# hpsim/OGL

Hardware: AMD Instinct MI355X
Metric: cg_iters_per_sec (higher is better)
Workload: dtype f64

## Files before the change

ogl_amd/csrc/kernels.hpp:

```cpp
#pragma once
#include <hip/hip_runtime.h>

#include "common.hpp"

namespace ogl {

struct DevCriterion {
    double tolerance, rel_tol;
    int32_t min_iter, max_iter, frequency, export_res;
};

struct DevScalars {
    double rho, prev_rho, beta;
    double alpha, omega, gamma;
    double norm_factor;
    double init_res, res;
    double xbar;
    double sums[4];
    int32_t iter;
    int32_t stop;
    int32_t n_evals;
    int32_t stop_phase;
    int32_t stop_turn;
    int32_t comm_error;
// ... 63 lines not shown
    const int32_t *chunk_bptr = nullptr;
    const int32_t *boundary_rows = nullptr;
    const int32_t *entry_ptrs = nullptr;
    const int32_t *cols = nullptr;
    const double *vals = nullptr;
    const double *recv = nullptr;
    const unsigned long long *local_flag = nullptr;
    int32_t n_neigh = 0;
    uint32_t seq = 0;
    long long timeout_ticks = 0;
    DevScalars *s = nullptr;
};
void launch_spmv(hipStream_t st, const DevCsr &A, int mode, const double *x, const double *b,
                 double *y, const SpmvDots &dots, const DevScalars *gate, const HaloFused &hf = HaloFused{});

struct DevEll {
    int32_t n_rows = 0;
    int32_t width = 0;
    int64_t stride = 0;
    const int32_t *cols = nullptr;
    const double *vals = nullptr;
    bool stream = false;
};
void launch_spmv_ell(hipStream_t st, const DevEll &A, int mode, const double *x, const double *b,
                     double *y, const SpmvDots &dots, const DevScalars *gate, const HaloFused &hf = HaloFused{});
struct DevSell {
    int32_t n_rows = 0;
    const SellChunk *chunks = nullptr;
    const int32_t *dict = nullptr;
    const uint8_t *codes = nullptr;
    const double *vals = nullptr;
    const int32_t *spill_chunk_ptr = nullptr, *spill_rows = nullptr, *spill_ptrs = nullptr, *spill_cols = nullptr;
    const double *spill_vals = nullptr;
    bool stream = false;
    int32_t xcd_group = 0;
    const uint16_t *rmap = nullptr;
    const int32_t *block_order = nullptr;
    int32_t n_blocks = 0;
};
void launch_spmv_sell(hipStream_t st, const DevSell &A, int mode, const double *x, const double *b,
                      double *y, const SpmvDots &dots, const DevScalars *gate, const HaloFused &hf = HaloFused{});
struct DevSym {
    int32_t n_rows = 0;
    int32_t nd = 0;
    int32_t d[4] = {0, 0, 0, 0};
    const uint8_t *mask = nullptr;
    const double *planes = nullptr;
    bool stream = false;
    const int32_t *block_order = nullptr;
    int32_t n_blocks = 0;
};
void launch_spmv_sym(hipStream_t st, const DevSym &A, int mode, const double *x, const double *b, double *y,
                     const SpmvDots &dots, const DevScalars *gate, const HaloFused &hf = HaloFused{});
struct DevSymx {
    int32_t n_rows = 0;
    const SymxChunk *chunks = nullptr, *chunks_general = nullptr;
    int32_t n_blocks_general = 0;
    const uint8_t *mask = nullptr;
    const double *planes = nullptr;
    const int32_t *ex_rowptr = nullptr, *ex_cols = nullptr;
    const int32_t *ex_lrow = nullptr;
    const double *ex_vals = nullptr;
    bool stream = false;
    bool fast = false;
    int32_t xcd_group = 0;
    int32_t n_blocks = 0;
};
void launch_spmv_symx(hipStream_t st, const DevSymx &A, int mode, const double *x, const double *b, double *y,
                      const SpmvDots &dots, const DevScalars *gate, const HaloFused &hf = HaloFused{});
void launch_gather_coeffs_masked(hipStream_t st, int64_t n, const int32_t *map, const double *source,
                                 double *out);
void launch_gather_sell(hipStream_t st, int32_t n_chunks, const SellChunk *chunks, const int32_t *map,
                        const double *source, double *out);

void launch_spmv_non_local(hipStream_t st, const DevHalo &H, int mode, const double *recv,
                           double *y, const DevScalars *gate);
void launch_pack(hipStream_t st, const DevHalo &H, const double *x, double *send,
                 const DevScalars *gate);

void launch_gather_coeffs(hipStream_t st, int32_t nnz, const int32_t *ldu_mapping,
                          const double *source, double *coeffs);
void launch_jacobi_generate(hipStream_t st, const DevCsr &A, double *inv_diag);
void launch_jacobi_generate_pos(hipStream_t st, const DevCsr &A, const int32_t *diag_pos, double *inv_diag);
void launch_jacobi_generate_diag(hipStream_t st, int32_t n_rows, const double *diag, double *inv_diag);

struct DevBlockJacobi {
    int32_t n_rows = 0;
    int32_t n_blocks = 0;
    int32_t stride = 0;
    const int32_t *block_ptrs = nullptr;
    const int32_t *row_block = nullptr;
    double *blocks = nullptr;
    int32_t uniform = 0;
    const int32_t *rows = nullptr, *pos = nullptr;
    int32_t by_device_row = 0;
    int32_t perm_xcd_group = 0;
};
constexpr int MAX_JACOBI_BLOCK = 32;
void launch_bj_generate(hipStream_t st, const DevCsr &A, const DevBlockJacobi &J,
                        bool group_lanes = true);
void launch_bj_apply(hipStream_t st, const DevBlockJacobi &J, const double *in, double *out,
                     double *dot_part, const DevScalars *gate);
void launch_bj_apply_staged(hipStream_t st, const DevBlockJacobi &J, const double *in, double *out, double *dot_part,
                            const DevScalars *gate, double *tmp_in, double *tmp_out);

constexpr int ISAI_THREAD_ROW = 32;
// ... 334 lines not shown
```

ogl_amd/csrc/kernels_spmv_sym.hip:

```cpp
#include <algorithm>

#include "device_common.hpp"
#include "resident_cg_turn.hpp"

namespace ogl {

namespace {

struct SymOffsets {
    int d[SYM_MAX_OFFSETS];
};
SymOffsets sym_offsets(const DevSym &A, bool *fast)
{
    SymOffsets off;
    for (int j = 0; j < SYM_MAX_OFFSETS; ++j) off.d[j] = A.d[j];
    *fast = A.nd >= 2 && A.d[1] == 1;
    for (int j = 2; j < A.nd; ++j) *fast = *fast && (A.d[j] % 2 == 0);
    return off;
}
template <int MODE, int ND, bool FAST, bool STREAM>
__device__ __forceinline__ double2 sym_rows(int chunk, const RowPair &rp, int n_rows, const SymOffsets &off,
                                            const uint8_t *__restrict__ mask, const double *__restrict__ planes,
                                            const double *__restrict__ x, const double *__restrict__ b,
                                            double2 &xd_out)
{
    const int t = threadIdx.x;
    const int row = rp.row;
    const unsigned mm = *reinterpret_cast<const unsigned short *>(mask + row);
    const unsigned m0 = mm & 0xffu, m1 = mm >> 8;
    double2 acc;
    acc.x = acc.y = 0.0;
    if (MODE == SPMV_RESIDUAL) acc = ld2(b, rp);
    double2 up[ND];
    const double *own = planes + (long)chunk * (ND * CHUNK_ROWS) + t * ROWS_PER_THREAD;
#pragma unroll
    for (int j = 0; j < ND; ++j)
        up[j] = (STREAM && (j == 0 || (FAST && j == 1))) ? ld_pair_stream(own + (long)j * CHUNK_ROWS)
                                                         : *reinterpret_cast<const double2 *>(own + (long)j * CHUNK_ROWS);
    const double2 xd = xd_out = ld2(x, rp);
    const int last = n_rows - 1, last_pair = last & ~1;
    double2 lo[ND];
#pragma unroll
    for (int j = 1; j < ND; ++j) {
        const int r0 = max(row - off.d[j], 0), r1 = max(row + 1 - off.d[j], 0);
        const long a0 = (long)(r0 >> 9) * (ND * CHUNK_ROWS) + (long)j * CHUNK_ROWS + (r0 & (CHUNK_ROWS - 1));
        const long a1 = (long)(r1 >> 9) * (ND * CHUNK_ROWS) + (long)j * CHUNK_ROWS + (r1 & (CHUNK_ROWS - 1));
        if (FAST && j >= 2) {
            lo[j] = *reinterpret_cast<const double2 *>(planes + a0);
        } else if (FAST) {
            if (STREAM) {
                lo[j].x = __shfl_up(up[1].y, 1, WAVE);
                if ((t & (WAVE - 1)) == 0) lo[j].x = planes[a0];
            } else {
                lo[j].x = planes[a0];
            }
            lo[j].y = up[1].x;
        } else {
            lo[j].x = planes[a0];
            lo[j].y = planes[a1];
        }
    }
    static_assert(CHUNK_ROWS == 512, "row >> 9 above");
    double2 xl[ND], xu[ND];
#pragma unroll
    for (int j = 1; j < ND; ++j) {
        if (FAST && j >= 2) {
            xl[j] = *reinterpret_cast<const double2 *>(x + min(max(row - off.d[j], 0), last_pair));
            xu[j] = *reinterpret_cast<const double2 *>(x + min(row + off.d[j], last_pair));
        } else if (FAST) {
            xl[j].x = x[min(max(row - 1, 0), last)];
            xl[j].y = xd.x;
            xu[j].x = xd.y;
            xu[j].y = x[min(row + 2, last)];
        } else {
            xl[j].x = x[min(max(row - off.d[j], 0), last)];
            xl[j].y = x[min(max(row + 1 - off.d[j], 0), last)];
            xu[j].x = x[min(row + off.d[j], last)];
            xu[j].y = x[min(row + 1 + off.d[j], last)];
        }
    }
#pragma unroll
    for (int j = ND - 1; j >= 1; --j) {
        if ((m0 >> (ND - 1 - j)) & 1u) {
            const double p = lo[j].x * xl[j].x;
            acc.x = (MODE == SPMV_RESIDUAL) ? acc.x - p : acc.x + p;
        }
        if ((m1 >> (ND - 1 - j)) & 1u) {
            const double p = lo[j].y * xl[j].y;
            acc.y = (MODE == SPMV_RESIDUAL) ? acc.y - p : acc.y + p;
        }
    }
    if ((m0 >> (ND - 1)) & 1u) {
        const double p = up[0].x * xd.x;
        acc.x = (MODE == SPMV_RESIDUAL) ? acc.x - p : acc.x + p;
    }
    if ((m1 >> (ND - 1)) & 1u) {
        const double p = up[0].y * xd.y;
        acc.y = (MODE == SPMV_RESIDUAL) ? acc.y - p : acc.y + p;
    }
#pragma unroll
    for (int j = 1; j < ND; ++j) {
        if ((m0 >> (ND - 1 + j)) & 1u) {
            const double p = up[j].x * xu[j].x;
            acc.x = (MODE == SPMV_RESIDUAL) ? acc.x - p : acc.x + p;
        }
        if ((m1 >> (ND - 1 + j)) & 1u) {
            const double p = up[j].y * xu[j].y;
            acc.y = (MODE == SPMV_RESIDUAL) ? acc.y - p : acc.y + p;
        }
    }
    return acc;
}

template <int MODE, int NDOT, int ND, bool FAST, bool STREAM>
__global__ __launch_bounds__(BLOCK) void k_spmv_sym(int n_rows, int n_chunks, SymOffsets off,
                                                    const uint8_t *__restrict__ mask,
                                                    const double *__restrict__ planes,
                                                    const double *__restrict__ x, const double *__restrict__ b,
                                                    double *__restrict__ y, const double *__restrict__ w,
                                                    double *__restrict__ dot_partials,
                                                    double *__restrict__ dot2_partials, const DevScalars *gate,
                                                    const int *__restrict__ block_order, HaloFused hf)
{
    __shared__ double slot[N_WAVES];
    __shared__ double ys[CHUNK_ROWS];
    if (gate && gate->stop) return;
    const int chunk = block_order ? block_order[blockIdx.x] : xcd_chunk(blockIdx.x);
    if (chunk < 0 || chunk >= n_chunks) return;
    const RowPair rp = my_rows(chunk, n_rows);
    double2 xd;
    double2 acc = sym_rows<MODE, ND, FAST, STREAM>(chunk, rp, n_rows, off, mask, planes, x, b, xd);
    if (hf.chunk_bptr) halo_fused_add<MODE>(hf, chunk, acc.x, acc.y, ys);
    st2(y, rp, acc);
    if (NDOT >= 1) {
        const double2 vw = ld2(w, rp);
        double d = 0.0, d2 = 0.0;
        if (rp.n > 0) {
            d += vw.x * acc.x;
            d2 += acc.x * acc.x;
        }
        if (rp.n > 1) {
            d += vw.y * acc.y;
            d2 += acc.y * acc.y;
        }
        const double s = block_sum(d, slot);
        if (threadIdx.x == 0) dot_partials[chunk] = s;
        if (NDOT >= 2) {
            const double s2 = block_sum(d2, slot);
            if (threadIdx.x == 0) dot2_partials[chunk] = s2;
        }
    }
}

template <int ND>
struct TurnSymRegs {
    double2 vd[2], vl[2][ND], vu[2][ND], up[ND], lo[ND];
};
template <int ND, bool FAST, bool STREAM>
__device__ __forceinline__ void turn_sym_load(TurnSymRegs<ND> &R, int chunk, const RowPair &rp, int n_rows,
                                              const SymOffsets &off, const double *__restrict__ planes,
                                              const double *__restrict__ p_in, const double *__restrict__ z)
{
    const int row = rp.row;
    const double *src[2] = {p_in, z};
    const int last = n_rows - 1, last_pair = last & ~1;
#pragma unroll
    for (int a = 0; a < 2; ++a) {
        const double *__restrict__ v = src[a];
        R.vd[a] = ld2(v, rp);
#pragma unroll
        for (int j = 1; j < ND; ++j) {
            if (FAST && j >= 2) {
                R.vl[a][j] = *reinterpret_cast<const double2 *>(v + min(max(row - off.d[j], 0), last_pair));
                R.vu[a][j] = *reinterpret_cast<const double2 *>(v + min(row + off.d[j], last_pair));
            } else if (FAST) {
                R.vl[a][j].x = v[min(max(row - 1, 0), last)];
                R.vl[a][j].y = R.vd[a].x;
                R.vu[a][j].x = R.vd[a].y;
                R.vu[a][j].y = v[min(row + 2, last)];
            } else {
                R.vl[a][j].x = v[min(max(row - off.d[j], 0), last)];
                R.vl[a][j].y = v[min(max(row + 1 - off.d[j], 0), last)];
                R.vu[a][j].x = v[min(row + off.d[j], last)];
                R.vu[a][j].y = v[min(row + 1 + off.d[j], last)];
            }
        }
    }
    const double *own = planes + (long)chunk * (ND * CHUNK_ROWS) + threadIdx.x * ROWS_PER_THREAD;
#pragma unroll
    for (int j = 0; j < ND; ++j)
        R.up[j] = (STREAM && (j == 0 || (FAST && j == 1))) ? ld_pair_stream(own + (long)j * CHUNK_ROWS)
                                                           : *reinterpret_cast<const double2 *>(own + (long)j * CHUNK_ROWS);
#pragma unroll
    for (int j = 1; j < ND; ++j) {
        const int r0 = max(row - off.d[j], 0), r1 = max(row + 1 - off.d[j], 0);
        const long a0 = (long)(r0 >> 9) * (ND * CHUNK_ROWS) + (long)j * CHUNK_ROWS + (r0 & (CHUNK_ROWS - 1));
        const long a1 = (long)(r1 >> 9) * (ND * CHUNK_ROWS) + (long)j * CHUNK_ROWS + (r1 & (CHUNK_ROWS - 1));
        if (FAST && j >= 2) {
            R.lo[j] = *reinterpret_cast<const double2 *>(planes + a0);
        } else if (FAST) {
            if (STREAM) {
                const double prev = __shfl_up(R.up[1].y, 1, WAVE);
// ... 292 lines not shown
    double beta;
    if (!turn_await_beta(a, ts, lds, beta)) return;
    resident_cg_turn<R, L, K>(src, a, ts, lds, z, f, beta);
}

}

void launch_spmv_sym(hipStream_t st, const DevSym &A, int mode, const double *x, const double *b, double *y,
                     const SpmvDots &dots, const DevScalars *gate, const HaloFused &hf)
{
    if (A.n_rows == 0) return;
    const int nc = (int)n_chunks(A.n_rows);
    const dim3 grid(A.block_order ? A.n_blocks : xcd_grid(nc)), block(BLOCK);
    bool fast;
    const SymOffsets off = sym_offsets(A, &fast);
#define OGL_SYM_K(MODE, NDOT, ND, FAST, STREAM)                                                                          \
    hipLaunchKernelGGL((k_spmv_sym<MODE, NDOT, ND, FAST, STREAM>), grid, block, 0, st, A.n_rows, nc, off, A.mask, A.planes, \
                       x, b, y, dots.with, dots.part, dots.part_yy, gate, A.block_order, hf)
#define OGL_SYM_ND(MODE, NDOT, ND)                   \
    do {                                             \
        if (fast && A.stream)                        \
            OGL_SYM_K(MODE, NDOT, ND, true, true);   \
        else if (fast)                               \
            OGL_SYM_K(MODE, NDOT, ND, true, false);  \
        else if (A.stream)                           \
            OGL_SYM_K(MODE, NDOT, ND, false, true);  \
        else                                         \
            OGL_SYM_K(MODE, NDOT, ND, false, false); \
    } while (0)
#define OGL_SYM(MODE, NDOT)                    \
    do {                                       \
        if (A.nd == 2)                         \
            OGL_SYM_ND(MODE, NDOT, 2);         \
        else if (A.nd == 3)                    \
            OGL_SYM_ND(MODE, NDOT, 3);         \
        else                                   \
            OGL_SYM_ND(MODE, NDOT, 4);         \
    } while (0)
    static_assert(SYM_MAX_OFFSETS == 4, "instantiations above");
    if (mode == SPMV_RESIDUAL) {
        OGL_SYM(SPMV_RESIDUAL, 0);
    } else if (dots.part && dots.part_yy) {
        OGL_SYM(SPMV_PLAIN, 2);
    } else if (dots.part) {
        OGL_SYM(SPMV_PLAIN, 1);
    } else {
        OGL_SYM(SPMV_PLAIN, 0);
    }
#undef OGL_SYM
#undef OGL_SYM_ND
#undef OGL_SYM_K
}

void launch_cg_turn_sym(hipStream_t st, const DevSym &A, const double *p_in, double *p_out, double *x, const double *z,
                        double *q, double *part_beta, const DevScalars *sin, DevScalars *sout,
                        const double *part_rho, const double *part_norm, double *history, int first, const LeadBox &lead)
{
    if (A.n_rows == 0) return;
    const int nc = (int)n_chunks(A.n_rows);
    const dim3 grid(A.block_order ? A.n_blocks : xcd_grid(nc)), block(BLOCK);
    const bool led = lead.box && nc >= 3 * FIN_WAVES;
    bool fast;
    const SymOffsets off = sym_offsets(A, &fast);
#define OGL_TURN_K(ND, FAST)                                                                                                  \
    do {                                                                                                                      \
        if (led)                                                                                                              \
            hipLaunchKernelGGL((k_cg_turn_sym<ND, FAST, true>), grid, block, 0, st, A.n_rows, nc, off, A.mask, A.planes, p_in, \
                               p_out, x, z, q, part_beta, sin, sout, part_rho, part_norm, nc, history, first, A.block_order,  \
                               lead);                                                                                         \
        else                                                                                                                  \
            hipLaunchKernelGGL((k_cg_turn_sym<ND, FAST, false>), grid, block, 0, st, A.n_rows, nc, off, A.mask, A.planes,     \
                               p_in, p_out, x, z, q, part_beta, sin, sout, part_rho, part_norm, nc, history, first,           \
                               A.block_order, LeadBox{});                                                                     \
    } while (0)
#define OGL_TURN_ND(ND)              \
    do {                             \
        if (fast)                    \
            OGL_TURN_K(ND, true);    \
        else                         \
            OGL_TURN_K(ND, false);   \
    } while (0)
    if (A.nd == 2)
        OGL_TURN_ND(2);
    else if (A.nd == 3)
        OGL_TURN_ND(3);
    else
        OGL_TURN_ND(4);
#undef OGL_TURN_ND
#undef OGL_TURN_K
}

void launch_cg_turn_sym_big(hipStream_t st, const DevSym &A, const double *p_in, double *p_out, double *x,
                            const double *z, double *q, double *part_beta, const DevScalars *s,
                            const HaloFused &hf, const double *p_halo_in, double *p_halo_out)
{
    if (A.n_rows == 0) return;
    const int nc = (int)n_chunks(A.n_rows);
    const dim3 grid(A.block_order ? A.n_blocks : xcd_grid(nc)), block(BLOCK);
    bool fast;
    const SymOffsets off = sym_offsets(A, &fast);
#define OGL_TURN_K(ND, FAST, STREAM)                                                                                \
    do {                                                                                                            \
        if (hf.chunk_bptr)                                                                                          \
            hipLaunchKernelGGL((k_cg_turn_sym_big<ND, FAST, STREAM, true>), grid, block, 0, st, A.n_rows, nc, off,  \
                               A.mask, A.planes, p_in, p_out, x, z, q, part_beta, s, A.block_order, hf, p_halo_in,  \
                               p_halo_out);                                                                         \
// ... 108 lines not shown
```

ogl_amd/csrc/solver.hpp:

```cpp
#pragma once
#include <hip/hip_runtime.h>

#include <algorithm>
#include <map>
#include <memory>
#include <string>
#include <vector>

#include "comm.hpp"
#include "common.hpp"
#include "host_matrix.hpp"
#include "kernels.hpp"
#include "setup_kernels.hpp"
#include "spmv_layouts.hpp"

namespace ogl {

struct MgLevel {
    int32_t n = 0, nnz = 0, n_coarse = 0;
    int passes = 0;
    bool own = true;
    DevBuf<int32_t> row_ptrs, cols;
    DevBuf<double> vals, inv_d;
    DevBuf<int32_t> agg, agg_ptr, agg_rows;
// ... 392 lines not shown
    std::vector<int32_t> fac_seg_fwd, fac_seg_bwd;
    ogl::DevBuf<double> d_part0, d_part1, d_part2;
    int64_t band_order_rows = 0;
    bool source_diag_valid = false;
    int64_t csr_band_rows = 0;
    uint64_t csr_band_pat = 0;
    int csr_band(int64_t *band);
    ogl::DevBuf<int32_t> d_band_order;
    ogl::DevBuf<double> d_part3, d_part4, d_part5;
    ogl::DevBuf<ogl::DevScalars> d_scal;
    ogl::DevBuf<double> d_history;
    ogl::DevScalars *h_scal = nullptr;
    hipEvent_t poll_ev[2] = {nullptr, nullptr};
    unsigned long long *lead_box = nullptr;
    unsigned long long *held_z_box = nullptr;
    size_t held_z_words = 0;
    int held_z_census = 0, held_z_census_grid = 0;
    unsigned *held_q_heads = nullptr;
    hipEvent_t chk_ev[2] = {nullptr, nullptr};
    bool x_resident = false, b_resident = false;
    ogl::PrecondData own_precond;
    const ogl::PrecondData *precond_data = nullptr;
    const double *precond = nullptr;

    std::map<std::string, double> props;

    std::vector<double> history;
    double t_update_matrix_ms = 0;
    std::vector<hipEvent_t> prof_ev;

    ~ogl_solver();

    int set_matrix(const ogl_ldu_view &ldu);
    int solve(const double *source, double *psi, ogl_perf *perf);
    int apply_resident(ogl_perf *perf);
    int upload_vec(ogl::DevBuf<double> &dst, const double *src);
    int ensure_vectors();
    int init_preconditioner();
    int generate_preconditioner(ogl::PrecondData &P);
    int generate_jacobi(ogl::PrecondData &P);
    int generate_block_jacobi(ogl::PrecondData &P, bool through_perm);
    int generate_isai(ogl::PrecondData &P, bool caller_numbering);
    int generate_factor(ogl::PrecondData &P);
    int prepare_apply();
    void apply_factor(const double *in, double *out, const ogl::DevScalars *gate, double *dot_part);
    int check_factor_breakdown(int32_t word);
    void apply_preconditioner(const double *in, double *out, const ogl::DevScalars *gate,
                              double *dot_part = nullptr);
    int dist_spmv(int mode, const double *x, const double *b, double *y, const ogl::SpmvDots &dots,
                  const ogl::DevScalars *gate, bool prepacked = false);
    void spmv_on(ogl::SpmvLayout l, int mode, const double *x, const double *b, double *y, const ogl::SpmvDots &dots,
                 const ogl::DevScalars *gate, const ogl::HaloFused &hf = ogl::HaloFused{});
    int finalize(int phase, ogl::FinArgs &a);
    int run_cg(ogl_perf *perf);
    int run_bicgstab(ogl_perf *perf);
    int run_krylov(ogl_perf *perf);
    ogl::MixedPart mixed;
    int mixed_requested(bool *on);
    int mixed_storage(const ogl::DevCriterion &crit, double inner_rel_tol, int inner_max_iter);
    int mixed_overflow(const ogl::MixedScalars &m);
    void mixed_spmv(const float *x, float *y, double *part, const ogl::MixedScalars *gate);
    int run_mixed(ogl_perf *perf);
    int ortho_requested(int *method);
    int spmv_f32(const float *x, float *y);
    struct KrylovRun;
    int krylov_plan(KrylovRun &k);
    int krylov_prepare(KrylovRun &k);
    int krylov_loop(KrylovRun &k);
    int krylov_enqueue(KrylovRun &k, int count);
    int krylov_finish(KrylovRun &k, ogl_perf *perf);
    int gmres_restart(KrylovRun &k, const ogl::DevScalars *gate);
    int gmres_update_x(KrylovRun &k, int cols, const ogl::DevScalars *gate);
    int turn_gmres(KrylovRun &k, int enq, int pe);
    int time_ortho_kernels(KrylovRun &k);
    int turn_cg_generic(KrylovRun &k, int enq, int pe);
    int turn_cg_generic_led(KrylovRun &k, int enq, int pe);
    int turn_cg_two_launch(KrylovRun &k, int enq, int pe);
    int turn_cg_three_launch(KrylovRun &k, int enq, int pe);
    int turn_cg_held_z(KrylovRun &k, int enq, int pe);
    int turn_cg_held_q(KrylovRun &k, int enq, int pe);
    int plan_held_z(KrylovRun &k);
    int turn_cg_merged(KrylovRun &k, int enq, int pe);
    int turn_cg_five_launch(KrylovRun &k, int enq, int pe);
    int turn_bicg_folded(KrylovRun &k, int enq, int pe);
    int turn_bicg(KrylovRun &k, int enq, int pe);
    int time_spmv(int repeats, double *avg_ms);
    ogl::DevHalo halo() const;
    double prop(const std::string &key, double dflt) const;
    const ogl_solver *share_from = nullptr;
    const double *offdiag_upper = nullptr, *offdiag_lower = nullptr;
    uint64_t offdiag_sum = 0;
    bool offdiag_valid = false;
    const ogl_label *seen_lower_addr = nullptr, *seen_upper_addr = nullptr;
    ogl_label seen_faces = -1;
    struct SeenIface {
        const ogl_label *face_cells;
        ogl_label size, kind, neighb_proc, neighb_patch;
    };
    std::vector<SeenIface> seen_iface_cells;
    bool saw_addressing(const ogl_ldu_view &ldu) const;
    bool peer_safe_wait() const;
    double stream_above_bytes() const;
    double turn_extra_bytes() const;
    int32_t xcd_group() const;
    int32_t pat_xcd_group = 0;
};
// ... 1 lines not shown
```

ogl_amd/csrc/solver_krylov.cpp:

```cpp
#include "launch_key.hpp"
#include "solver_internal.hpp"

#include <algorithm>
#include <cmath>
#include <cstring>
#include <vector>

using namespace ogl;

HaloPutFused ogl_solver::begin_halo_put()
{
    HaloPutFused put;
    if (!(pat.non_local_nnz > 0 && peer_halo) || prop("haloFused", 1.0) == 0.0 || peer_safe_wait())
        return put;
    if (++halo_seq == 0) ++halo_seq;
    cur_halo = peer_halo_args(halo_seq);
    put.P = cur_halo;
    put.chunk_sptr = d_chunk_sptr.p;
    put.send_pos = d_send_pos.p;
    put.send_idxs = d_send_idxs.p;
    put.ticket = d_ticket.p;
    put.n_put_chunks = n_put_chunks;
    return put;
}
// ... 219 lines not shown
                       prop("fusedFinalizers", 1.0) != 0.0;
    const bool lead_any = !multi && !small && nc >= 3 * 16 && prop("leadFinalizers", 1.0) != 0.0;
    const bool lead_ok = lead_any && !bicg && !gmres;
    bool fused = k.fused = !bicg && !gmres && ((small && !generic) || lead_ok);
    k.lead = LeadBox{};
    k.s2 = s + 1;
    k.bicg_fold = bicg && (small || lead_any) && prop("bicgFold", 1.0) != 0.0;
    OGL_TRY(ortho_requested(&k.ortho));
    props["orthoMethodInUse"] = (double)k.ortho;
    k.gmres_fold = gmres && !k.ortho && (small || (lead_any && prop("gmresLead", 0.0) != 0.0)) && prop("gmresFold", 1.0) != 0.0;
    if (gmres)
        props["gmresLaunchesPerTurn"] =
            2.0 + (k.ortho ? 2.0 + 2.0 * k.ortho : k.gmres_fold ? 0.5 * (k.m - 1) + 3.0 : (double)(k.m - 1) + 4.0);
    k.slot_s[0] = s;
    k.slot_s[1] = k.s2;
    props["fusedFinalizersInUse"] = ((fused || k.bicg_fold || k.gmres_fold) && small) ? 1.0 : 0.0;
    bool merged = !bicg && !gmres && !generic && nc >= 1 && spmv_layout == SpmvLayout::Sym &&
                  ((fused && small) ? prop("fusedTurn", 1.0) != 0.0 : prop("fusedTurnBig", sym().stream ? 0.0 : 1.0) != 0.0);
    if (multi)
        merged = merged && peer_halo && prop("haloFused", 1.0) != 0.0 && prop("fusedTurnMulti", 1.0) != 0.0 &&
                 !peer_safe_wait();
    k.n_global = (double)n;
    if (multi) {
        const double mine[2] = {(double)n, merged ? 0.0 : 1.0};
        double got[2] = {0.0, 0.0};
        OGL_HIP_CHECK(hipMemcpyAsync(sums_ptr(s), mine, sizeof(mine), hipMemcpyHostToDevice, st));
        OGL_HIP_CHECK(hipStreamSynchronize(st));
        OGL_TRY(reg->allreduce(sums_ptr(s), 2));
        OGL_HIP_CHECK(hipMemcpyAsync(got, sums_ptr(s), sizeof(got), hipMemcpyDeviceToHost, st));
        OGL_HIP_CHECK(hipStreamSynchronize(st));
        k.n_global = got[0];
        merged = got[1] == 0.0;
    }
    if ((lead_ok && fused) || (lead_any && (k.bicg_fold || k.gmres_fold))) {
        if (!lead_box) {
            void *b = nullptr;
            OGL_HIP_CHECK(ledger::dev_malloc(&b, LEAD_REPLICAS * LEAD_REPLICA_STRIDE * sizeof(unsigned long long), true));
            lead_box = static_cast<unsigned long long *>(b);
        }
        OGL_HIP_CHECK(hipMemsetAsync(lead_box, 0, LEAD_REPLICAS * LEAD_REPLICA_STRIDE * sizeof(unsigned long long), st));
        k.lead.box = lead_box;
        k.lead.timeout_ticks = (long long)(prop("leadTimeoutS", 10.0) * 1e8);
        k.lead.early_loads = prop("leadEarlyLoads", 1.0) != 0.0 ? 1 : 0;
    }
    props["leadFinalizersInUse"] = k.lead.box ? 1.0 : 0.0;
    props["fusedFinalizersInUse"] = ((fused || k.bicg_fold || k.gmres_fold) && small) ? 1.0 : 0.0;
    k.merged = merged;
    k.fused2 = fused && merged;
    k.merged_halo = merged && multi && pat.non_local_nnz > 0;
    props["fusedTurnInUse"] = merged ? 1.0 : 0.0;
    return OGL_OK;
}

int ogl_solver::krylov_prepare(KrylovRun &k)
{
    hipStream_t st = k.st;
    const int n = k.n, nc = k.nc, m = k.m;
    DevScalars *s = k.s;
    const bool bicg = k.bicg, gmres = k.gmres, generic = k.generic, merged = k.merged;
    int ring_k = 0;
    if (k.lead.box != nullptr && k.fused && !k.fused2 && prop("deferX2", 1.0) != 0.0) {
        const double want = prop("deferX", 2.0);
        ring_k = want >= 8.0 ? 8 : want >= 4.0 ? 4 : want >= 2.0 ? 2 : 0;
    }
    props["deferXInUse"] = (double)ring_k;
    props["deferX2InUse"] = ring_k ? 1.0 : 0.0;
    if (merged || ring_k) OGL_TRY(d_p2.alloc((size_t)n + 2, st));
    for (int i = 2; i < ring_k; ++i) OGL_TRY(d_pring[i - 2].alloc((size_t)n + 2, st));
    if (merged && precond) OGL_TRY(d_z.alloc((size_t)n + 2, st));
    k.n_halo = (size_t)pat.non_local_nnz;
    if (k.merged_halo) {
        OGL_TRY(d_p_halo.alloc(2 * k.n_halo + 2, st));
        OGL_HIP_CHECK(hipMemsetAsync(d_p_halo.p, 0, d_p_halo.n * sizeof(double), st));
    }
    k.p0 = d_p.p;
    k.p1 = d_p2.p;
    k.ring.k = ring_k;
    for (int i = 0; i < ring_k; ++i) k.ring.b[i] = i == 0 ? d_p.p : i == 1 ? d_p2.p : d_pring[i - 2].p;
    k.ph = d_p_halo.p;
    k.z_kept = merged && precond ? d_z.p : nullptr;
    OGL_TRY(plan_held_z(k));

    k.is_final = cfg.rel_tol == 0.0;
    const int prev_iters = (int)prop(k.is_final ? "prevSolveIters_final" : "prevSolveIters", 1);
    const double prev_cost = prop("_prev_solve", 0.0);
    DevCriterion &crit = k.crit;
    crit.tolerance = cfg.tolerance;
    crit.rel_tol = cfg.rel_tol;
    crit.max_iter = bicg ? 2 * cfg.max_iter : cfg.max_iter;
    crit.export_res = cfg.export_res;
    ogl_host_adapt_criterion(&cfg, prev_iters, prev_cost, &crit.min_iter, &crit.frequency);
    if (crit.frequency < 1) return fail(OGL_ERR_INVALID, "evalFrequency must be >= 1");
    k.max_checks = std::max(crit.max_iter, crit.min_iter) + crit.frequency + 1;
    k.max_turns = bicg ? k.max_checks / 2 + 1 : k.max_checks;
    OGL_TRY(d_history.alloc((size_t)std::max(k.max_checks, crit.max_iter + std::max(1, cfg.norm_eval_limit) + 1) + 4, st));
    if (cfg.export_res)
        OGL_HIP_CHECK(hipMemsetAsync(d_history.p, 0, d_history.n * sizeof(double), st));
    if (k.bicg_fold) {
        OGL_TRY(d_part3.alloc((size_t)nc, st));
        OGL_TRY(d_part4.alloc((size_t)nc, st));
        OGL_TRY(d_part5.alloc((size_t)nc, st));
    }
    if (bicg) {
        const size_t nv = (size_t)n + 2;
        OGL_TRY(d_v.alloc(nv, st));
        OGL_TRY(d_s.alloc(nv, st));
        OGL_TRY(d_t.alloc(nv, st));
        OGL_TRY(d_rr.alloc(nv, st));
        if (precond || generic) {
            OGL_TRY(d_y.alloc(nv, st));
            OGL_TRY(d_z.alloc(nv, st));
        }
    } else if (gmres) {
        OGL_TRY(d_V.alloc((size_t)(m + 1) * (size_t)k.ldv, st));
        OGL_TRY(d_gm.alloc(gmres_state_len(m), st));
        OGL_HIP_CHECK(hipMemsetAsync(d_gm.p, 0, gmres_state_len(m) * sizeof(double), st));
        if (generic) OGL_TRY(d_z.alloc((size_t)n + 2, st));
        if (k.ortho) {
            OGL_TRY(d_gs_part.alloc((size_t)(m + 1) * (size_t)nc, st));
            OGL_TRY(d_gs_h.alloc((size_t)m + 1, st));
        }
    } else if (generic) {
        OGL_TRY(d_z.alloc((size_t)n + 2, st));
    }

    k.prof_stride = std::max(0, cfg.profile_kernels);
    k.prof_cap = k.prof_stride ? std::min((k.max_turns + k.prof_stride - 1) / k.prof_stride, 4096) : 0;
    while ((int)prof_ev.size() < 2 * k.prof_cap) {
        hipEvent_t e;
        OGL_HIP_CHECK(ev_create(&e));
        prof_ev.push_back(e);
    }
    for (int i = 0; i < 2; ++i) {
        if (!chk_ev[i]) OGL_HIP_CHECK(ev_create(&chk_ev[i]));
        k.ev_chk[i] = chk_ev[i];
    }

    k.t_start = now_ms();
    launch_reset_scalars(st, s, crit);

    FinArgs fa;
    launch_partials_sum(st, n, d_x.p, d_part0.p);
    fa = FinArgs{};
    fa.part[0] = d_part0.p;
    fa.n_part = nc;
    fa.n_sums = 1;
    fa.n_local = (double)n;
    fa.n_global = k.n_global;
    OGL_TRY(finalize(FIN_MEAN, fa));
    launch_fill_xbar(st, n, d_w.p, s);
    OGL_TRY(dist_spmv(SPMV_PLAIN, d_w.p, nullptr, d_q.p, SpmvDots{}, nullptr));
    OGL_TRY(dist_spmv(SPMV_RESIDUAL, d_x.p, d_b.p, d_r.p, SpmvDots{}, nullptr));
    launch_partials_normfactor(st, n, d_b.p, d_q.p, d_r.p, d_part0.p);
    fa = FinArgs{};
    fa.part[0] = d_part0.p;
    fa.n_part = nc;
    fa.n_sums = 1;
    OGL_TRY(finalize(FIN_NORMFACTOR, fa));

    OGL_HIP_CHECK(hipMemsetAsync(d_p.p, 0, (size_t)n * sizeof(double), st));
    k.fg = FinArgs{};
    k.fg.part[0] = d_part0.p;
    k.fg.part[1] = d_part1.p;
    k.fg.n_part = nc;
    k.fg.history = d_history.p;
    k.fg.gm = d_gm.p;
    k.fg.m = m;
    k.beta_ptr = reinterpret_cast<const double *>(reinterpret_cast<const char *>(s) + offsetof(DevScalars, beta));
    k.gm = d_gm.p;
    k.gm_y = d_gm.p + (size_t)(m + 1) * m + 2 * (size_t)m + (m + 1);
    if (gmres) {
        OGL_HIP_CHECK(hipEventRecord(k.ev_chk[0], st));
        OGL_TRY(gmres_restart(k, nullptr));
        OGL_HIP_CHECK(hipEventRecord(k.ev_chk[1], st));
    } else if (bicg) {
        OGL_HIP_CHECK(hipMemcpyAsync(d_rr.p, d_r.p, (size_t)n * sizeof(double),
                                     hipMemcpyDeviceToDevice, st));
        OGL_HIP_CHECK(hipMemsetAsync(d_v.p, 0, (size_t)n * sizeof(double), st));
        launch_cg_rho_norm(st, n, d_r.p, nullptr, d_part0.p, d_part1.p, s);
    } else {
        launch_cg_rho_norm(st, n, d_r.p, precond, d_part0.p, d_part1.p, s);
        if (k.z_kept) launch_mul(st, n, k.z_kept, d_r.p, precond, nullptr);
        if (generic) {
            apply_preconditioner(d_r.p, d_z.p, s, d_part0.p);
        }
    }
    k.chk = FinArgs{};
    k.chk.part[0] = d_part0.p;
    k.chk.part[1] = d_part1.p;
    k.chk.n_part = nc;
    k.chk.n_sums = 2;
    k.chk.history = d_history.p;
    if (!gmres && !k.folded()) {
        OGL_HIP_CHECK(hipEventRecord(k.ev_chk[0], st));
        OGL_TRY(finalize(FIN_CG_CHECK, k.chk));
        OGL_HIP_CHECK(hipEventRecord(k.ev_chk[1], st));
    }
    if (k.merged_halo) {
        if (++halo_seq == 0) ++halo_seq;
        cur_halo = peer_halo_args(halo_seq);
        launch_pack_put_signal(st, halo(), cur_halo, k.z_kept ? k.z_kept : d_r.p, s, d_ticket.p);
    }

    k.f1 = FinArgs{};
    k.f1.part[0] = d_part0.p;
    k.f1.n_part = nc;
    k.f1.n_sums = 1;
    k.f1.history = d_history.p;
    k.f2 = k.f1;
    k.f2.part[1] = d_part1.p;
    k.f2.n_sums = 2;

    k.y = (precond || generic) ? d_y.p : d_p.p;
    k.z = (precond || generic) ? d_z.p : d_s.p;
    k.enq = 0;
    return OGL_OK;
}

int ogl_solver::gmres_restart(KrylovRun &k, const DevScalars *gate)
{
    launch_cg_rho_norm(k.st, k.n, d_r.p, nullptr, d_part0.p, d_part1.p, gate);
    k.fg.n_sums = 2;
    k.fg.check_after = gate ? 0 : 1;
    OGL_TRY(finalize(FIN_GMRES_RESTART, k.fg));
    k.fg.check_after = 0;
    if (!k.gmres_scale_late()) launch_gmres_scale(k.st, k.n, d_V.p, d_r.p, k.beta_ptr, gate);
    return OGL_OK;
}

int ogl_solver::gmres_update_x(KrylovRun &k, int cols, const DevScalars *gate)
{
    if (cols <= 0) return OGL_OK;
    k.fg.n_sums = 0;
    k.fg.turn = cols;
// ... 716 lines not shown
```

ogl_amd/csrc/solver_mixed.cpp:

```cpp
#include "solver_internal.hpp"

#include <algorithm>
#include <climits>
#include <cmath>
#include <vector>

using namespace ogl;

namespace {

const char *solver_name(int kind)
{
    return kind == OGL_SOLVER_CG ? "GKOCG" : kind == OGL_SOLVER_BICGSTAB ? "GKOBiCGStab" : "GKOGMRES";
}

int32_t *word_of(MixedScalars *m, size_t offset) { return reinterpret_cast<int32_t *>(reinterpret_cast<char *>(m) + offset); }

}

int ogl_solver::mixed_requested(bool *on)
{
    *on = prop("mixedPrecision", 0.0) != 0.0;
    if (!*on) return OGL_OK;
    const double inner_rel_tol = prop("innerRelTol", 1e-4), inner_max_iter = prop("innerMaxIter", 1000.0);
// ... 40 lines not shown
        launch_mixed_spmv_csr(reg->stream, csr(false), fp32_dev.vals.p, x, y, part, gate);
}

int ogl_solver::mixed_overflow(const MixedScalars &m)
{
    if (m.bad_coef == INT_MAX && m.bad_invd == INT_MAX) return OGL_OK;
    fp32_dev.epoch = 0;
    const bool coef = m.bad_coef != INT_MAX;
    int64_t row = m.bad_invd;
    if (coef && fp32_dev.half) {
        const int64_t per_chunk = (int64_t)sym_dev.nd * CHUNK_ROWS;
        row = (m.bad_coef / per_chunk) * CHUNK_ROWS + m.bad_coef % CHUNK_ROWS;
    } else if (coef) {
        std::vector<int32_t> rp((size_t)pat.n_rows + 1);
        OGL_HIP_CHECK(hipMemcpy(rp.data(), d_row_ptrs.p, rp.size() * sizeof(int32_t), hipMemcpyDeviceToHost));
        row = (int64_t)(std::upper_bound(rp.begin(), rp.end(), m.bad_coef) - rp.begin()) - 1;
    }
    row = std::max<int64_t>(0, std::min<int64_t>(row, (int64_t)pat.n_rows - 1));
    if (pat.renumbered() && (size_t)row < pat.old_of.size()) row = pat.old_of[(size_t)row];
    return fail(OGL_ERR_INVALID, "mixedPrecision: %s of row %lld is finite in double precision and not in single precision",
                coef ? "a coefficient" : "the inverse diagonal", (long long)row);
}

int ogl_solver::run_mixed(ogl_perf *perf)
{
    hipStream_t st = reg->stream;
    const int n = pat.n_rows, nc = (int)n_chunks(n);
    DevScalars *s = d_scal.p;
    const bool is_final = cfg.rel_tol == 0.0;
    DevCriterion crit{};
    crit.tolerance = cfg.tolerance;
    crit.rel_tol = cfg.rel_tol;
    crit.min_iter = cfg.min_iter;
    crit.max_iter = cfg.max_iter;
    crit.frequency = 1;
    crit.export_res = cfg.export_res;
    const int inner_max_iter = (int)std::min(prop("innerMaxIter", 1000.0), 2147483647.0);
    OGL_TRY(mixed_storage(crit, prop("innerRelTol", 1e-4), inner_max_iter));
    MixedScalars *m = mixed.scal.p;
    const float *inv_d = nullptr;
    if (precond) {
        launch_mixed_refresh(st, n, nullptr, precond, mixed.inv_d.p, word_of(m, offsetof(MixedScalars, bad_invd)));
        inv_d = mixed.inv_d.p;
    }
    float *z = inv_d ? mixed.z.p : mixed.r.p;
    OGL_TRY(d_history.alloc((size_t)std::max(std::max(crit.max_iter, crit.min_iter) + 2,
                                             crit.max_iter + std::max(1, cfg.norm_eval_limit) + 1) + 4, st));
    if (cfg.export_res) OGL_HIP_CHECK(hipMemsetAsync(d_history.p, 0, d_history.n * sizeof(double), st));
    for (int i = 0; i < 2; ++i)
        if (!chk_ev[i]) OGL_HIP_CHECK(ev_create(&chk_ev[i]));

    const double t_start = now_ms();
    launch_reset_scalars(st, s, crit);
    launch_partials_sum(st, n, d_x.p, d_part0.p);
    FinArgs fa{};
    fa.part[0] = d_part0.p;
    fa.n_part = nc;
    fa.n_sums = 1;
    fa.n_local = fa.n_global = (double)n;
    OGL_TRY(finalize(FIN_MEAN, fa));
    launch_fill_xbar(st, n, d_w.p, s);
    OGL_TRY(dist_spmv(SPMV_PLAIN, d_w.p, nullptr, d_q.p, SpmvDots{}, nullptr));
    OGL_TRY(dist_spmv(SPMV_RESIDUAL, d_x.p, d_b.p, d_r.p, SpmvDots{}, nullptr));
    launch_partials_normfactor(st, n, d_b.p, d_q.p, d_r.p, d_part0.p);
    fa = FinArgs{};
    fa.part[0] = d_part0.p;
    fa.n_part = nc;
    fa.n_sums = 1;
    OGL_TRY(finalize(FIN_NORMFACTOR, fa));
    launch_partials_norm1(st, n, d_r.p, d_part2.p);

    auto poll_record = [&](int slot) -> int {
        OGL_HIP_CHECK(hipMemcpyAsync(&mixed.h_scal[slot], m, sizeof(MixedScalars), hipMemcpyDeviceToHost, st));
        OGL_HIP_CHECK(hipEventRecord(poll_ev[slot], st));
        return OGL_OK;
    };
    auto enqueue_turns = [&](int count) {
        for (int i = 0; i < count; ++i) {
            launch_mixed_step1(st, n, mixed.p.p, z, m);
            mixed_spmv(mixed.p.p, mixed.q.p, d_part2.p, m);
            launch_mixed_fin_pi(st, m, d_part2.p, nc);
            launch_mixed_step2(st, n, mixed.u.p, mixed.r.p, mixed.p.p, mixed.q.p, inv_d, mixed.z.p, d_part0.p, d_part1.p, m);
        }
    };
    const int batch = 16;
    int turns = 0, enqueued = 0;
    MixedScalars fin{};
    for (int k = 0;; ++k) {
        if (k == 0) OGL_HIP_CHECK(hipEventRecord(chk_ev[0], st));
        launch_mixed_head(st, m, s, d_part2.p, nc, d_history.p);
        if (k == 0) OGL_HIP_CHECK(hipEventRecord(chk_ev[1], st));
        launch_mixed_start(st, n, d_r.p, inv_d, mixed.r.p, z, mixed.u.p, d_part0.p, d_part1.p, m);
        const int cap = std::max(0, std::min(inner_max_iter, crit.max_iter - turns));
        int enq = 0;
        auto next_batch = [&]() {
            const int count = std::min(batch, cap - enq);
            enqueue_turns(count);
            enq += count;
            enqueued += count;
        };
        next_batch();
        OGL_TRY(poll_record(0));
        MixedScalars seen{};
        for (int j = 0;; ++j) {
            const bool more = enq < cap;
            if (more) {
                next_batch();
                OGL_TRY(poll_record((j + 1) & 1));
            }
            OGL_HIP_CHECK(hipEventSynchronize(poll_ev[j & 1]));
            seen = mixed.h_scal[j & 1];
            if (seen.outer_stop || seen.inner_stop) break;
            if (!more) return fail(OGL_ERR_STATE, "mixedPrecision: the inner solve did not stop within its budget");
        }
        if (seen.outer_stop) {
            fin = seen;
            break;
        }
        turns += seen.inner_turns;
        launch_mixed_add(st, n, d_x.p, mixed.u.p, m);
        OGL_TRY(dist_spmv(SPMV_RESIDUAL, d_x.p, d_b.p, d_r.p, SpmvDots{}, s));
        launch_partials_norm1(st, n, d_r.p, d_part2.p);
// ... 76 lines not shown
```

Measured before the change: 5077.

## Fuse CG solve prologue into one symmetric SpMV kernel with reductions

Adds a fused prologue kernel for the symmetric SpMV layout. It computes the residual r = b - Ax, the row sums of A times the mean xbar (replacing the fill_xbar vector and the second SpMV), the norm-factor partials, and optionally the initial rho and norm partials, all in one pass. This removes several kernel launches and full-vector passes (w fill, A*w SpMV, separate normfactor and rho/norm kernels) from the per-solve setup. It only applies to single-device Sym layout without non-local entries, and it adds register pressure and extra block reductions to the prologue kernel.

```diff
diff --git a/ogl_amd/csrc/kernels.hpp b/ogl_amd/csrc/kernels.hpp
--- a/ogl_amd/csrc/kernels.hpp
+++ b/ogl_amd/csrc/kernels.hpp
@@ -139,6 +139,8 @@
 };
 void launch_spmv_sym(hipStream_t st, const DevSym &A, int mode, const double *x, const double *b, double *y,
                      const SpmvDots &dots, const DevScalars *gate, const HaloFused &hf = HaloFused{});
+void launch_prologue_sym(hipStream_t st, const DevSym &A, const double *x, const double *b, double *r,
+                         const double *inv_diag, double *part_nf, double *part_rho, double *part_norm, const DevScalars *s);
 struct DevSymx {
     int32_t n_rows = 0;
     const SymxChunk *chunks = nullptr, *chunks_general = nullptr;
diff --git a/ogl_amd/csrc/kernels_spmv_sym.hip b/ogl_amd/csrc/kernels_spmv_sym.hip
--- a/ogl_amd/csrc/kernels_spmv_sym.hip
+++ b/ogl_amd/csrc/kernels_spmv_sym.hip
@@ -18,11 +18,11 @@
     for (int j = 2; j < A.nd; ++j) *fast = *fast && (A.d[j] % 2 == 0);
     return off;
 }
-template <int MODE, int ND, bool FAST, bool STREAM>
+template <int MODE, int ND, bool FAST, bool STREAM, bool QBAR = false>
 __device__ __forceinline__ double2 sym_rows(int chunk, const RowPair &rp, int n_rows, const SymOffsets &off,
                                             const uint8_t *__restrict__ mask, const double *__restrict__ planes,
                                             const double *__restrict__ x, const double *__restrict__ b,
-                                            double2 &xd_out)
+                                            double2 &xd_out, double xbar = 0.0, double2 *qbar = nullptr)
 {
     const int t = threadIdx.x;
     const int row = rp.row;
@@ -79,36 +79,45 @@
             xu[j].y = x[min(row + 1 + off.d[j], last)];
         }
     }
+    double2 qb;
+    qb.x = qb.y = 0.0;
 #pragma unroll
     for (int j = ND - 1; j >= 1; --j) {
         if ((m0 >> (ND - 1 - j)) & 1u) {
             const double p = lo[j].x * xl[j].x;
             acc.x = (MODE == SPMV_RESIDUAL) ? acc.x - p : acc.x + p;
+            if (QBAR) qb.x = qb.x + lo[j].x * xbar;
         }
         if ((m1 >> (ND - 1 - j)) & 1u) {
             const double p = lo[j].y * xl[j].y;
             acc.y = (MODE == SPMV_RESIDUAL) ? acc.y - p : acc.y + p;
+            if (QBAR) qb.y = qb.y + lo[j].y * xbar;
         }
     }
     if ((m0 >> (ND - 1)) & 1u) {
         const double p = up[0].x * xd.x;
         acc.x = (MODE == SPMV_RESIDUAL) ? acc.x - p : acc.x + p;
+        if (QBAR) qb.x = qb.x + up[0].x * xbar;
     }
     if ((m1 >> (ND - 1)) & 1u) {
         const double p = up[0].y * xd.y;
         acc.y = (MODE == SPMV_RESIDUAL) ? acc.y - p : acc.y + p;
+        if (QBAR) qb.y = qb.y + up[0].y * xbar;
     }
 #pragma unroll
     for (int j = 1; j < ND; ++j) {
         if ((m0 >> (ND - 1 + j)) & 1u) {
             const double p = up[j].x * xu[j].x;
             acc.x = (MODE == SPMV_RESIDUAL) ? acc.x - p : acc.x + p;
+            if (QBAR) qb.x = qb.x + up[j].x * xbar;
         }
         if ((m1 >> (ND - 1 + j)) & 1u) {
             const double p = up[j].y * xu[j].y;
             acc.y = (MODE == SPMV_RESIDUAL) ? acc.y - p : acc.y + p;
-        }
-    }
+            if (QBAR) qb.y = qb.y + up[j].y * xbar;
+        }
+    }
+    if (QBAR) *qbar = qb;
     return acc;
 }
 
@@ -148,6 +157,66 @@
         if (NDOT >= 2) {
             const double s2 = block_sum(d2, slot);
             if (threadIdx.x == 0) dot2_partials[chunk] = s2;
+        }
+    }
+}
+
+template <bool RHO, int ND, bool FAST, bool STREAM>
+__global__ __launch_bounds__(BLOCK) void k_prologue_sym(int n_rows, int n_chunks, SymOffsets off,
+                                                        const uint8_t *__restrict__ mask,
+                                                        const double *__restrict__ planes,
+                                                        const double *__restrict__ x, const double *__restrict__ b,
+                                                        double *__restrict__ r, const double *__restrict__ inv_diag,
+                                                        double *__restrict__ part_nf, double *__restrict__ part_rho,
+                                                        double *__restrict__ part_norm, const DevScalars *s,
+                                                        const int *__restrict__ block_order)
+{
+    __shared__ double slot[N_WAVES];
+    const int chunk = block_order ? block_order[blockIdx.x] : xcd_chunk(blockIdx.x);
+    if (chunk < 0 || chunk >= n_chunks) return;
+    const double xbar = s->xbar;
+    const RowPair rp = my_rows(chunk, n_rows);
+    const double2 vb = ld2(b, rp);
+    double2 vi;
+    vi.x = vi.y = 1.0;
+    if (RHO && inv_diag) vi = ld2(inv_diag, rp);
+    double2 xd, vw;
+    const double2 vr =
+        sym_rows<SPMV_RESIDUAL, ND, FAST, STREAM, true>(chunk, rp, n_rows, off, mask, planes, x, b, xd, xbar, &vw);
+    st2(r, rp, vr);
+    double e = 0.0;
+    if (rp.n > 0) {
+        const double t = vb.x - 1.0 * vw.x;
+        const double p2 = fabs(t);
+        e += fabs(fabs(t - 1.0 * vr.x) + 1.0 * p2);
+    }
+    if (rp.n > 1) {
+        const double t = vb.y - 1.0 * vw.y;
+        const double p2 = fabs(t);
+        e += fabs(fabs(t - 1.0 * vr.y) + 1.0 * p2);
+    }
+    const double se = block_sum(e, slot);
+    if (threadIdx.x == 0) part_nf[chunk] = se;
+    if (RHO) {
+        double2 vz = vr;
+        if (inv_diag) {
+            vz.x = vr.x * vi.x;
+            vz.y = vr.y * vi.y;
+        }
+        double d = 0.0, a = 0.0;
+        if (rp.n > 0) {
+            d += vr.x * vz.x;
+            a += fabs(vr.x);
+        }
+        if (rp.n > 1) {
+            d += vr.y * vz.y;
+            a += fabs(vr.y);
+        }
+        const double s0 = block_sum(d, slot);
+        const double s1 = block_sum(a, slot);
+        if (threadIdx.x == 0) {
+            part_rho[chunk] = s0;
+            part_norm[chunk] = s1;
         }
     }
 }
@@ -546,6 +615,47 @@
 #undef OGL_SYM_K
 }
 
+void launch_prologue_sym(hipStream_t st, const DevSym &A, const double *x, const double *b, double *r,
+                         const double *inv_diag, double *part_nf, double *part_rho, double *part_norm, const DevScalars *s)
+{
+    if (A.n_rows == 0) return;
+    const int nc = (int)n_chunks(A.n_rows);
+    const dim3 grid(A.block_order ? A.n_blocks : xcd_grid(nc)), block(BLOCK);
+    bool fast;
+    const SymOffsets off = sym_offsets(A, &fast);
+#define OGL_PRO_K(RHO, ND, FAST, STREAM)                                                                                  \
+    hipLaunchKernelGGL((k_prologue_sym<RHO, ND, FAST, STREAM>), grid, block, 0, st, A.n_rows, nc, off, A.mask, A.planes, x, \
+                       b, r, inv_diag, part_nf, part_rho, part_norm, s, A.block_order)
+#define OGL_PRO_ND(RHO, ND)                   \
+    do {                                      \
+        if (fast && A.stream)                 \
+            OGL_PRO_K(RHO, ND, true, true);   \
+        else if (fast)                        \
+            OGL_PRO_K(RHO, ND, true, false);  \
+        else if (A.stream)                    \
+            OGL_PRO_K(RHO, ND, false, true);  \
+        else                                  \
+            OGL_PRO_K(RHO, ND, false, false); \
+    } while (0)
+#define OGL_PRO(RHO)                \
+    do {                            \
+        if (A.nd == 2)              \
+            OGL_PRO_ND(RHO, 2);     \
+        else if (A.nd == 3)         \
+            OGL_PRO_ND(RHO, 3);     \
+        else                        \
+            OGL_PRO_ND(RHO, 4);     \
+    } while (0)
+    static_assert(SYM_MAX_OFFSETS == 4, "instantiations above");
+    if (part_rho)
+        OGL_PRO(true);
+    else
+        OGL_PRO(false);
+#undef OGL_PRO
+#undef OGL_PRO_ND
+#undef OGL_PRO_K
+}
+
 void launch_cg_turn_sym(hipStream_t st, const DevSym &A, const double *p_in, double *p_out, double *x, const double *z,
                         double *q, double *part_beta, const DevScalars *sin, DevScalars *sout,
                         const double *part_rho, const double *part_norm, double *history, int first, const LeadBox &lead)
diff --git a/ogl_amd/csrc/solver.hpp b/ogl_amd/csrc/solver.hpp
--- a/ogl_amd/csrc/solver.hpp
+++ b/ogl_amd/csrc/solver.hpp
@@ -468,6 +468,7 @@
     void spmv_on(ogl::SpmvLayout l, int mode, const double *x, const double *b, double *y, const ogl::SpmvDots &dots,
                  const ogl::DevScalars *gate, const ogl::HaloFused &hf = ogl::HaloFused{});
     int finalize(int phase, ogl::FinArgs &a);
+    int solve_prologue(double n_global, bool first_sums, const double *inv_diag);
     int run_cg(ogl_perf *perf);
     int run_bicgstab(ogl_perf *perf);
     int run_krylov(ogl_perf *perf);
diff --git a/ogl_amd/csrc/solver_krylov.cpp b/ogl_amd/csrc/solver_krylov.cpp
--- a/ogl_amd/csrc/solver_krylov.cpp
+++ b/ogl_amd/csrc/solver_krylov.cpp
@@ -295,6 +295,42 @@
     return OGL_OK;
 }
 
+int ogl_solver::solve_prologue(double n_global, bool first_sums, const double *inv_diag)
+{
+    hipStream_t st = reg->stream;
+    const int n = pat.n_rows, nc = (int)n_chunks(n);
+    DevScalars *s = d_scal.p;
+    const bool materialised_z = precond_data && precond_data->materialises_z();
+    const bool fused = prop("fusedPrologue", 1.0) != 0.0 && spmv_layout == SpmvLayout::Sym && !reg->comm->multi() &&
+                       pat.non_local_nnz == 0 && (!first_sums || !materialised_z);
+    props["fusedPrologueInUse"] = fused ? 1.0 : 0.0;
+    launch_partials_sum(st, n, d_x.p, d_part0.p);
+    FinArgs fa{};
+    fa.part[0] = d_part0.p;
+    fa.n_part = nc;
+    fa.n_sums = 1;
+    fa.n_local = (double)n;
+    fa.n_global = n_global;
+    OGL_TRY(finalize(FIN_MEAN, fa));
+    fa = FinArgs{};
+    fa.n_part = nc;
+    fa.n_sums = 1;
+    if (fused) {
+        launch_prologue_sym(st, sym(), d_x.p, d_b.p, d_r.p, inv_diag, d_part2.p, first_sums ? d_part0.p : nullptr,
+                            first_sums ? d_part1.p : nullptr, s);
+        fa.part[0] = d_part2.p;
+        return finalize(FIN_NORMFACTOR, fa);
+    }
+    launch_fill_xbar(st, n, d_w.p, s);
+    OGL_TRY(dist_spmv(SPMV_PLAIN, d_w.p, nullptr, d_q.p, SpmvDots{}, nullptr));
+    OGL_TRY(dist_spmv(SPMV_RESIDUAL, d_x.p, d_b.p, d_r.p, SpmvDots{}, nullptr));
+    launch_partials_normfactor(st, n, d_b.p, d_q.p, d_r.p, d_part0.p);
+    fa.part[0] = d_part0.p;
+    OGL_TRY(finalize(FIN_NORMFACTOR, fa));
+    if (first_sums) launch_cg_rho_norm(st, n, d_r.p, inv_diag, d_part0.p, d_part1.p, s);
+    return OGL_OK;
+}
+
 int ogl_solver::krylov_prepare(KrylovRun &k)
 {
     hipStream_t st = k.st;
@@ -382,24 +418,8 @@
     k.t_start = now_ms();
     launch_reset_scalars(st, s, crit);
 
-    FinArgs fa;
-    launch_partials_sum(st, n, d_x.p, d_part0.p);
-    fa = FinArgs{};
-    fa.part[0] = d_part0.p;
-    fa.n_part = nc;
-    fa.n_sums = 1;
-    fa.n_local = (double)n;
-    fa.n_global = k.n_global;
-    OGL_TRY(finalize(FIN_MEAN, fa));
-    launch_fill_xbar(st, n, d_w.p, s);
-    OGL_TRY(dist_spmv(SPMV_PLAIN, d_w.p, nullptr, d_q.p, SpmvDots{}, nullptr));
-    OGL_TRY(dist_spmv(SPMV_RESIDUAL, d_x.p, d_b.p, d_r.p, SpmvDots{}, nullptr));
-    launch_partials_normfactor(st, n, d_b.p, d_q.p, d_r.p, d_part0.p);
-    fa = FinArgs{};
-    fa.part[0] = d_part0.p;
-    fa.n_part = nc;
-    fa.n_sums = 1;
-    OGL_TRY(finalize(FIN_NORMFACTOR, fa));
+    const bool first_sums = !gmres;
+    OGL_TRY(solve_prologue(k.n_global, first_sums, bicg ? nullptr : precond));
 
     OGL_HIP_CHECK(hipMemsetAsync(d_p.p, 0, (size_t)n * sizeof(double), st));
     k.fg = FinArgs{};
@@ -420,9 +440,7 @@
         OGL_HIP_CHECK(hipMemcpyAsync(d_rr.p, d_r.p, (size_t)n * sizeof(double),
                                      hipMemcpyDeviceToDevice, st));
         OGL_HIP_CHECK(hipMemsetAsync(d_v.p, 0, (size_t)n * sizeof(double), st));
-        launch_cg_rho_norm(st, n, d_r.p, nullptr, d_part0.p, d_part1.p, s);
     } else {
-        launch_cg_rho_norm(st, n, d_r.p, precond, d_part0.p, d_part1.p, s);
         if (k.z_kept) launch_mul(st, n, k.z_kept, d_r.p, precond, nullptr);
         if (generic) {
             apply_preconditioner(d_r.p, d_z.p, s, d_part0.p);
diff --git a/ogl_amd/csrc/solver_mixed.cpp b/ogl_amd/csrc/solver_mixed.cpp
--- a/ogl_amd/csrc/solver_mixed.cpp
+++ b/ogl_amd/csrc/solver_mixed.cpp
@@ -116,22 +116,7 @@
 
     const double t_start = now_ms();
     launch_reset_scalars(st, s, crit);
-    launch_partials_sum(st, n, d_x.p, d_part0.p);
-    FinArgs fa{};
-    fa.part[0] = d_part0.p;
-    fa.n_part = nc;
-    fa.n_sums = 1;
-    fa.n_local = fa.n_global = (double)n;
-    OGL_TRY(finalize(FIN_MEAN, fa));
-    launch_fill_xbar(st, n, d_w.p, s);
-    OGL_TRY(dist_spmv(SPMV_PLAIN, d_w.p, nullptr, d_q.p, SpmvDots{}, nullptr));
-    OGL_TRY(dist_spmv(SPMV_RESIDUAL, d_x.p, d_b.p, d_r.p, SpmvDots{}, nullptr));
-    launch_partials_normfactor(st, n, d_b.p, d_q.p, d_r.p, d_part0.p);
-    fa = FinArgs{};
-    fa.part[0] = d_part0.p;
-    fa.n_part = nc;
-    fa.n_sums = 1;
-    OGL_TRY(finalize(FIN_NORMFACTOR, fa));
+    OGL_TRY(solve_prologue((double)n, false, nullptr));
     launch_partials_norm1(st, n, d_r.p, d_part2.p);
 
     auto poll_record = [&](int slot) -> int {
```

New measurement: 5124 (median of 4 runs). About the same (+0.9%).
